# uc-vision/smart-tree

Hardware: AMD Instinct MI355X
Metric: points/sec end-to-end (voxelize->sparse-UNet->skeleton), 1M-pt tree (higher is better)
Workload: dtype f32

## Files before the change

### smart_tree_amd/csrc/brick.hip

```cpp
#include "st_common.h"
#include "st_grid.h"

#define BK_BLOCK 256
#define BK_MAX_DEPTH 6

struct alignas(16) BkRec {
    unsigned long long mask[8];
    unsigned char cum[8];
    unsigned tidx;
    unsigned cum_hi;
};

struct BkLevel {
    int mb;
    unsigned mt;
    int64_t ntab;
    uint32_t* p;
    BkRec* rec;
    uint32_t* base;
    int64_t slot_cap;
    int64_t* n_slots;
    int64_t* n_vox;
};

struct BkState {
    int ext[ST_MAX_SEG][3];
    unsigned fail;
};

__device__ __forceinline__ unsigned bk_spread3(unsigned v) {
    v &= 0x7fu;
    v = (v | (v << 8)) & 0x0000700fu;
    v = (v | (v << 4)) & 0x000430c3u;
    v = (v | (v << 2)) & 0x00049249u;
    return v;
}
__device__ __forceinline__ unsigned bk_compact3(unsigned v) {
    v &= 0x00049249u;
    v = (v | (v >> 2)) & 0x000430c3u;
    v = (v | (v >> 4)) & 0x0000700fu;
    v = (v | (v >> 8)) & 0x0000007fu;
    return v;
}
__device__ __forceinline__ unsigned bk_morton(int bz, int by, int bx) { return (bk_spread3((unsigned)bz) << 2) | (bk_spread3((unsigned)by) << 1) | bk_spread3((unsigned)bx); }
__device__ __forceinline__ unsigned bk_cum(const BkRec& r, int w) { return (unsigned)r.cum[w] + (((r.cum_hi >> w) & 1u) << 8); }

__device__ __forceinline__ int64_t bk_tab(const BkLevel& L, int b, int z, int y, int x) {
    return (int64_t)b * L.mt + bk_morton(z >> 3, y >> 3, x >> 3);
}
__device__ __forceinline__ int bk_lookup(const BkLevel& L, int b, int z, int y, int x) {
    const int lim = 8 << L.mb;
    if ((unsigned)z >= (unsigned)lim || (unsigned)y >= (unsigned)lim || (unsigned)x >= (unsigned)lim) return -1;
    const int64_t t = bk_tab(L, b, z, y, x);
    const uint32_t s = L.p[t];
    if (L.p[t + 1] == s) return -1;
    const BkRec& r = L.rec[s];
    const int w = z & 7, bit = ((y & 7) << 3) | (x & 7);
    const unsigned long long m = r.mask[w];
    if (!((m >> bit) & 1ull)) return -1;
    return (int)(L.base[s] + bk_cum(r, w) + (unsigned)__popcll(m & ((1ull << bit) - 1ull)));
}

#define BK_LOOP(i, n) for (int64_t i = (int64_t)blockIdx.x * blockDim.x + threadIdx.x; i < (n); i += (int64_t)gridDim.x * blockDim.x)

static inline unsigned bk_grid(int64_t n) {
    int64_t g = st_div_up(n > 0 ? n : 1, BK_BLOCK);
    return (unsigned)(g < 16384 ? g : 16384);
}

__global__ void __launch_bounds__(BK_BLOCK) k_bk_mark0(const int32_t* coords, int64_t n, BkLevel L, BkState* st, const int32_t* blk_seg,
                                                       int nseg, int nblk) {
    __shared__ int m[ST_MAX_SEG * 3];
    for (int i = threadIdx.x; i < nseg * 3; i += blockDim.x) m[i] = 0;
    __syncthreads();
    const int lim = 8 << L.mb;
    BK_LOOP(i, n) {
        const int4 c = reinterpret_cast<const int4*>(coords)[i];
        if ((unsigned)c.x >= (unsigned)nblk || (unsigned)c.y >= (unsigned)lim || (unsigned)c.z >= (unsigned)lim || (unsigned)c.w >= (unsigned)lim) {
            atomicOr(&st->fail, 2u);
            continue;
        }
        L.p[bk_tab(L, c.x, c.y, c.z, c.w)] = 1u;
        const int s = blk_seg ? blk_seg[c.x] : 0;
        if (c.y > m[3 * s]) atomicMax(&m[3 * s], c.y);
        if (c.z > m[3 * s + 1]) atomicMax(&m[3 * s + 1], c.z);
        if (c.w > m[3 * s + 2]) atomicMax(&m[3 * s + 2], c.w);
    }
    __syncthreads();
    for (int i = threadIdx.x; i < nseg * 3; i += blockDim.x) if (m[i]) atomicMax(&(&st->ext[0][0])[i], m[i]);
}

__global__ void __launch_bounds__(BK_BLOCK) k_bk_init_rec(BkLevel L, BkState* st) {
    BK_LOOP(t, L.ntab) {
        const uint32_t s = L.p[t];
        if (L.p[t + 1] == s) continue;
        if ((int64_t)s >= L.slot_cap) { atomicOr(&st->fail, 1u); continue; }
        BkRec r;
#pragma unroll
        for (int w = 0; w < 8; w++) { r.mask[w] = 0ull; r.cum[w] = 0; }
        r.tidx = (unsigned)t;
        r.cum_hi = 0u;
        L.rec[s] = r;
    }
}

__device__ __forceinline__ void bk_set_bit(const BkLevel& L, int b, int z, int y, int x) {
    const uint32_t s = L.p[bk_tab(L, b, z, y, x)];
    if ((int64_t)s >= L.slot_cap) return;
    const int bit = ((y & 7) << 3) | (x & 7);
    unsigned* half = reinterpret_cast<unsigned*>(&L.rec[s].mask[z & 7]) + (bit >> 5);
    const unsigned v = 1u << (bit & 31);
    if (!(*half & v)) atomicOr(half, v);
}

__global__ void __launch_bounds__(BK_BLOCK) k_bk_bits0(const int32_t* coords, int64_t n, BkLevel L, const BkState* st) {
    if (st->fail) return;
    const int lim = 8 << L.mb;
    BK_LOOP(i, n) {
        const int4 c = reinterpret_cast<const int4*>(coords)[i];
        if ((unsigned)c.y >= (unsigned)lim || (unsigned)c.z >= (unsigned)lim || (unsigned)c.w >= (unsigned)lim) continue;
        bk_set_bit(L, c.x, c.y, c.z, c.w);
    }
}

__global__ void __launch_bounds__(BK_BLOCK) k_bk_count(BkLevel L) {
    const int64_t ns = *L.n_slots < L.slot_cap ? *L.n_slots : L.slot_cap;
    BK_LOOP(s, ns) {
        BkRec& r = L.rec[s];
        unsigned run = 0, hi = 0;
#pragma unroll
        for (int w = 0; w < 8; w++) {
            r.cum[w] = (unsigned char)(run & 255u);
            hi |= (run >> 8) << w;
            run += (unsigned)__popcll(r.mask[w]);
        }
        r.cum_hi = hi;
        L.base[s] = run;
    }
}

__global__ void __launch_bounds__(BK_BLOCK) k_bk_order0(const int32_t* coords, int64_t n, BkLevel L, int32_t* order0, int32_t* sorted,
                                                        const BkState* st) {
    if (st->fail) return;
    BK_LOOP(i, n) {
        const int4 c = reinterpret_cast<const int4*>(coords)[i];
        const int r = bk_lookup(L, c.x, c.y, c.z, c.w);
        if (r < 0 || r >= n) continue;
        order0[r] = (int32_t)i;
        reinterpret_cast<int4*>(sorted)[r] = c;
    }
}

__global__ void __launch_bounds__(BK_BLOCK) k_bk_subm(const int32_t* coords, const int64_t* n_dev, int64_t cap, BkLevel L, int32_t* nbr,
                                                      const BkState* st) {
    if (st->fail) return;
    const int64_t n = *n_dev < cap ? *n_dev : cap;
    const int lim = 8 << L.mb;
    BK_LOOP(o, n) {
        const int4 c = reinterpret_cast<const int4*>(coords)[o];
        const int b = c.x, z = c.y, y = c.z, x = c.w;
        int slot[8];
        uint32_t bs[8];
#pragma unroll
        for (int q = 0; q < 8; q++) {
            const int zz = z + ((q & 4) ? 1 : -1), yy = y + ((q & 2) ? 1 : -1), xx = x + ((q & 1) ? 1 : -1);
            slot[q] = -1;
            bs[q] = 0u;
            if ((unsigned)zz < (unsigned)lim && (unsigned)yy < (unsigned)lim && (unsigned)xx < (unsigned)lim) {
                const int64_t t = bk_tab(L, b, zz, yy, xx);
                const uint32_t s = L.p[t];
                if (L.p[t + 1] != s) { slot[q] = (int)s; bs[q] = L.base[s]; }
            }
        }
#pragma unroll
        for (int dz = -1; dz <= 1; dz++) {
            const int zz = z + dz, w = zz & 7;
            const int qz = (zz >> 3) == ((z - 1) >> 3) ? 0 : 4;
            unsigned long long m[4];
            unsigned cu[4];
#pragma unroll
            for (int q = 0; q < 4; q++) {
                const int s = slot[qz | q];
                m[q] = 0ull;
                cu[q] = 0u;
                if (s >= 0 && (unsigned)zz < (unsigned)lim) { const BkRec& r = L.rec[s]; m[q] = r.mask[w]; cu[q] = bs[qz | q] + bk_cum(r, w); }
            }
#pragma unroll
            for (int j = 0; j < 9; j++) {
                const int dy = j / 3 - 1, dx = j % 3 - 1;
                const int yy = y + dy, xx = x + dx, k = (dz + 1) * 9 + j;
                int r = -1;
                if (dz == 0 && j == 4) r = (int)o;
                else if ((unsigned)yy < (unsigned)lim && (unsigned)xx < (unsigned)lim) {
                    const int q = ((yy >> 3) == ((y - 1) >> 3) ? 0 : 2) | ((xx >> 3) == ((x - 1) >> 3) ? 0 : 1);
                    const int bit = ((yy & 7) << 3) | (xx & 7);
                    const unsigned long long mm = m[q];
                    if ((mm >> bit) & 1ull) r = (int)(cu[q] + (unsigned)__popcll(mm & ((1ull << bit) - 1ull)));
                }
                nbr[(int64_t)k * cap + o] = r;
            }
        }
    }
}

__global__ void __launch_bounds__(BK_BLOCK) k_bk_coarse_mark(BkLevel Lf, BkLevel Lc, const BkState* st, int level, const int32_t* blk_seg) {
    if (st->fail) return;
    const int64_t ns = *Lf.n_slots < Lf.slot_cap ? *Lf.n_slots : Lf.slot_cap;
    const int nbc = 1 << Lc.mb;
    BK_LOOP(s, ns) {
        const BkRec& r = Lf.rec[s];
        const unsigned t = r.tidx, mc = t & (Lf.mt - 1u);
        const int b = (int)(t >> (3 * Lf.mb));
        const int fb[3] = {(int)bk_compact3(mc >> 2), (int)bk_compact3(mc >> 1), (int)bk_compact3(mc)};
        const int* e = st->ext[blk_seg ? blk_seg[b] : 0];
        unsigned long long all = 0ull;
#pragma unroll
        for (int w = 0; w < 8; w++) all |= r.mask[w];
        for (int q = 0; q < 8; q++) {
            const int d[3] = {(q >> 2) & 1, (q >> 1) & 1, q & 1};
            unsigned long long m = d[0] ? r.mask[7] : all;
            if (d[1]) m &= 0xff00000000000000ull;
            if (d[2]) m &= 0x8080808080808080ull;
            bool ok = m != 0ull;
            int cb[3];
#pragma unroll
            for (int a = 0; a < 3; a++) {
                cb[a] = (fb[a] >> 1) + d[a];
                ok = ok && (!d[a] || (fb[a] & 1)) && cb[a] < nbc && 8 * cb[a] <= ((e[a] >> level) >> 1);
            }
            if (ok) Lc.p[(int64_t)b * Lc.mt + bk_morton(cb[0], cb[1], cb[2])] = 1u;
        }
    }
}

__global__ void __launch_bounds__(BK_BLOCK) k_bk_coarse_stencil(BkLevel Lf, BkLevel Lc, const BkState* st, int level, const int32_t* blk_seg) {
    if (st->fail) return;
    const int64_t ns = *Lc.n_slots < Lc.slot_cap ? *Lc.n_slots : Lc.slot_cap;
    const int limf = 8 << Lf.mb, nbf = 1 << Lf.mb;
    BK_LOOP(idx, ns * 8) {
        const int64_t s = idx >> 3;
        const int w = (int)(idx & 7);
        const unsigned t = Lc.rec[s].tidx, mc = t & (Lc.mt - 1u);
        const int b = (int)(t >> (3 * Lc.mb));
        const int cb[3] = {(int)bk_compact3(mc >> 2), (int)bk_compact3(mc >> 1), (int)bk_compact3(mc)};
        const int* e = st->ext[blk_seg ? blk_seg[b] : 0];
        const int omax[3] = {(e[0] >> level) >> 1, (e[1] >> level) >> 1, (e[2] >> level) >> 1};
        const int oz = 8 * cb[0] + w;
        unsigned long long word = 0ull;
        if (oz <= omax[0]) {
            unsigned rows[17];
#pragma unroll
            for (int r = 0; r < 17; r++) rows[r] = 0u;
            for (int dz = -1; dz <= 1; dz++) {
                const int fz = 2 * oz + dz;
                if (fz < 0 || fz >= limf) continue;
                const int fbz = fz >> 3, wz = fz & 7;
                for (int iy = 0; iy < 3; iy++) {
                    const int fby = 2 * cb[1] - 1 + iy;
                    if (fby < 0 || fby >= nbf) continue;
                    for (int ix = 0; ix < 3; ix++) {
                        const int fbx = 2 * cb[2] - 1 + ix;
                        if (fbx < 0 || fbx >= nbf) continue;
                        const int64_t tf = (int64_t)b * Lf.mt + bk_morton(fbz, fby, fbx);
                        const uint32_t sf = Lf.p[tf];
                        if (Lf.p[tf + 1] == sf) continue;
                        const unsigned long long m = Lf.rec[sf].mask[wz];
                        if (m == 0ull) continue;
                        for (int yy = iy == 0 ? 7 : 0; yy < 8; yy++) {
                            const unsigned rb = (unsigned)(m >> (8 * yy)) & 0xffu;
                            const int r = iy == 0 ? 0 : (iy == 1 ? 1 + yy : 9 + yy);
                            rows[r] |= ix == 0 ? (rb >> 7) : (ix == 1 ? rb << 1 : rb << 9);
                        }
                    }
                }
            }
            unsigned c8[17];
#pragma unroll
            for (int r = 0; r < 17; r++) {
                unsigned x = rows[r] | (rows[r] >> 1) | (rows[r] >> 2);
                x &= 0x5555u;
                x = (x | (x >> 1)) & 0x3333u;
                x = (x | (x >> 2)) & 0x0f0fu;
                x = (x | (x >> 4)) & 0x00ffu;
                c8[r] = x;
            }
            unsigned xclip = 0xffu;
            if (8 * cb[2] + 7 > omax[2]) xclip = omax[2] >= 8 * cb[2] ? (0xffu >> (7 - (omax[2] - 8 * cb[2]))) : 0u;
#pragma unroll
            for (int oy = 0; oy < 8; oy++) {
                if (8 * cb[1] + oy > omax[1]) break;
                const unsigned rb = (c8[2 * oy] | c8[2 * oy + 1] | c8[2 * oy + 2]) & xclip;
                word |= (unsigned long long)rb << (8 * oy);
            }
        }
        Lc.rec[s].mask[w] = word;
    }
}

__global__ void __launch_bounds__(BK_BLOCK) k_bk_emit(BkLevel L, int32_t* coords, int64_t cap, BkState* st) {
    if (st->fail) return;
    const int64_t ns = *L.n_slots < L.slot_cap ? *L.n_slots : L.slot_cap;
    BK_LOOP(idx, ns * 8) {
        const int64_t s = idx >> 3;
        const int w = (int)(idx & 7);
        const BkRec& r = L.rec[s];
        unsigned long long m = r.mask[w];
        if (m == 0ull) continue;
        const unsigned t = r.tidx, mc = t & (L.mt - 1u);
        const int b = (int)(t >> (3 * L.mb));
        const int z = (int)(bk_compact3(mc >> 2) << 3) | w, y0 = (int)(bk_compact3(mc >> 1) << 3), x0 = (int)(bk_compact3(mc) << 3);
        int64_t row = (int64_t)L.base[s] + bk_cum(r, w);
        while (m) {
            const int bit = __ffsll((long long)m) - 1;
            m &= m - 1ull;
            if (row < cap) reinterpret_cast<int4*>(coords)[row] = make_int4(b, z, y0 + (bit >> 3), x0 + (bit & 7));
            else atomicOr(&st->fail, 1u);
            row++;
        }
    }
}

__device__ __forceinline__ int bk_parity_class(int z, int y, int x) { return ((z & 1) << 2) | ((y & 1) << 1) | (x & 1); }
__global__ void __launch_bounds__(BK_BLOCK) k_bk_updown(const int32_t* coords, const int64_t* n_dev, int64_t cap_f, BkLevel Lc, const BkState* st,
                                                        int level, const int32_t* blk_seg, const int64_t* m_dev, int64_t cap_c,
                                                        int32_t* nbr_up, int32_t* nbr_down, uint32_t* parity_count) {
    __shared__ uint32_t hist[8];
    if (st->fail) return;
    if (threadIdx.x < 8) hist[threadIdx.x] = 0;
    __syncthreads();
    const int64_t n = *n_dev < cap_f ? *n_dev : cap_f;
    const int64_t m = *m_dev < cap_c ? *m_dev : cap_c;
    BK_LOOP(i, n) {
        const int4 c4 = reinterpret_cast<const int4*>(coords)[i];
        const int b = c4.x, c[3] = {c4.y, c4.z, c4.w};
        const int* e = st->ext[blk_seg ? blk_seg[b] : 0];
        const int omax[3] = {(e[0] >> level) >> 1, (e[1] >> level) >> 1, (e[2] >> level) >> 1};
        atomicAdd(&hist[bk_parity_class(c[0], c[1], c[2])], 1u);
        int64_t t_have = -1;
        int slot = -1, w_have = -1;
        unsigned bs = 0u, cu = 0u;
        unsigned long long mw = 0ull;
        const int limc = 8 << Lc.mb;
#pragma unroll
        for (int kz = 0; kz < 3; kz++)
#pragma unroll
            for (int j = 0; j < 9; j++) {
                const int k = kz * 9 + j;
                const int nz = c[0] + 1 - kz, ny = c[1] + 1 - j / 3, nx = c[2] + 1 - j % 3;
                int r = -1;
                if (!((nz | ny | nx) & 1) && nz >= 0 && ny >= 0 && nx >= 0 && (nz >> 1) <= omax[0] && (ny >> 1) <= omax[1] && (nx >> 1) <= omax[2]) {
                    const int oz = nz >> 1, oy = ny >> 1, ox = nx >> 1;
                    if (oz < limc && oy < limc && ox < limc) {
                        const int64_t tc = bk_tab(Lc, b, oz, oy, ox);
                        if (tc != t_have) {
                            t_have = tc;
                            w_have = -1;
                            const uint32_t sc = Lc.p[tc];
                            slot = Lc.p[tc + 1] != sc ? (int)sc : -1;
                            bs = slot >= 0 ? Lc.base[slot] : 0u;
                        }
                        if (slot >= 0) {
                            const int wz = oz & 7;
                            if (wz != w_have) { w_have = wz; const BkRec& rc = Lc.rec[slot]; mw = rc.mask[wz]; cu = bs + bk_cum(rc, wz); }
                            const int bit = ((oy & 7) << 3) | (ox & 7);
                            if ((mw >> bit) & 1ull) r = (int)(cu + (unsigned)__popcll(mw & ((1ull << bit) - 1ull)));
                        }
                    }
                }
                nbr_up[(int64_t)k * cap_f + i] = r;
                if (r >= 0 && r < m) nbr_down[(int64_t)k * cap_c + r] = (int32_t)i;
            }
    }
    __syncthreads();
    if (threadIdx.x < 8 && hist[threadIdx.x]) atomicAdd(&parity_count[threadIdx.x], hist[threadIdx.x]);
}

#define BK_ORDER_BLOCKS 512
__global__ void __launch_bounds__(BK_BLOCK) k_bk_parity_order(const int32_t* coords, const int64_t* n_dev, int64_t cap, const uint32_t* count,
                                                              uint32_t* cursor, int32_t* order, const BkState* st) {
    __shared__ uint32_t hist[8], gbase[8], lcur[8];
    if (st->fail) return;
    const int64_t n = *n_dev < cap ? *n_dev : cap;
    const int lane = threadIdx.x & 63;
    const int64_t per = (n + gridDim.x - 1) / gridDim.x, chunk = (per + BK_BLOCK - 1) / BK_BLOCK * BK_BLOCK;
    const int64_t lo = (int64_t)blockIdx.x * chunk, hi = lo + chunk < n ? lo + chunk : n;
    if (threadIdx.x < 8) { hist[threadIdx.x] = 0; lcur[threadIdx.x] = 0; }
    __syncthreads();
    for (int64_t i0 = lo + (threadIdx.x - lane); i0 < hi; i0 += BK_BLOCK) {
        const int64_t i = i0 + lane;
        int cls = -1;
        if (i < hi) cls = bk_parity_class(coords[4 * i + 1], coords[4 * i + 2], coords[4 * i + 3]);
        for (int q = 0; q < 8; q++) {
            const unsigned long long mask = __ballot(cls == q);
            if (mask != 0ull && lane == __ffsll((long long)mask) - 1) atomicAdd(&hist[q], (uint32_t)__popcll(mask));
        }
    }
    __syncthreads();
    if (threadIdx.x < 8) {
        uint32_t base = 0;
        for (int q = 0; q < (int)threadIdx.x; q++) base += count[q];
        gbase[threadIdx.x] = base + (hist[threadIdx.x] ? atomicAdd(&cursor[threadIdx.x], hist[threadIdx.x]) : 0u);
    }
    __syncthreads();
    for (int64_t i0 = lo + (threadIdx.x - lane); i0 < hi; i0 += BK_BLOCK) {
        const int64_t i = i0 + lane;
        int cls = -1;
        if (i < hi) cls = bk_parity_class(coords[4 * i + 1], coords[4 * i + 2], coords[4 * i + 3]);
        for (int q = 0; q < 8; q++) {
            const unsigned long long mask = __ballot(cls == q);
            if (mask == 0ull) continue;
            const int leader = __ffsll((long long)mask) - 1;
            uint32_t at = 0;
            if (lane == leader) at = atomicAdd(&lcur[q], (uint32_t)__popcll(mask));
            at = __shfl(at, leader);
            if (cls == q)
                order[gbase[q] + at + (uint32_t)__popcll(mask & ((1ull << lane) - 1ull))] = (int32_t)((uint32_t)i | ((8u + (uint32_t)q) << 28));
        }
    }
}

struct BkPlan {
    int depth;
    int mb[BK_MAX_DEPTH + 1];
    int64_t ntab[BK_MAX_DEPTH + 1], slot_cap[BK_MAX_DEPTH + 1];
};

static bool bk_plan(int64_t n0, int n_blocks, int coord_bound, int depth, const int64_t* caps, BkPlan* P) {
    if (depth < 0 || depth > BK_MAX_DEPTH || n_blocks < 1 || coord_bound < 1) return false;
    P->depth = depth;
    int bound = coord_bound;
    for (int l = 0; l <= depth; l++) {
        int nb = (bound + 7) / 8, mb = 0;
        while ((1 << mb) < nb) mb++;
        if (mb > 7) return false;
        P->mb[l] = mb;
        P->ntab[l] = (int64_t)n_blocks << (3 * mb);
        if (P->ntab[l] >= (1ll << 31)) return false;
        const int64_t cap = l == 0 ? n0 : caps[l];
        P->slot_cap[l] = cap < P->ntab[l] ? cap : P->ntab[l];
        bound = (bound - 1) / 2 + 1;
    }
    return true;
}

struct BkLayout {
    BkState* st;
    int64_t* counts;
    uint32_t* p[BK_MAX_DEPTH + 1];
    BkRec* rec[BK_MAX_DEPTH + 1];
    uint32_t* base[BK_MAX_DEPTH + 1];
    char* scan_ws;
    int64_t scan_bytes;
};

static void bk_layout(StArena& a, const BkPlan& P, BkLayout* Y) {
    Y->st = a.take<BkState>(1);
    Y->counts = a.take<int64_t>(2 * (BK_MAX_DEPTH + 1));
    int64_t scan_n = 1;
    for (int l = 0; l <= P.depth; l++) {
        Y->p[l] = a.take<uint32_t>(P.ntab[l] + 1);
        Y->rec[l] = a.take<BkRec>(P.slot_cap[l]);
        Y->base[l] = a.take<uint32_t>(P.slot_cap[l] + 1);
        if (P.ntab[l] + 1 > scan_n) scan_n = P.ntab[l] + 1;
        if (P.slot_cap[l] + 1 > scan_n) scan_n = P.slot_cap[l] + 1;
    }
    Y->scan_bytes = st_scan_ws_bytes(scan_n);
    Y->scan_ws = a.take<char>(Y->scan_bytes);
}

extern "C" int64_t st_brick_pyramid_workspace_bytes(int64_t n0, int n_blocks, int coord_bound, int depth, const int64_t* caps) {
    BkPlan P;
    if (!bk_plan(n0 > 0 ? n0 : 1, n_blocks, coord_bound, depth, caps, &P)) return 0;
    StArena a(nullptr, 0);
    BkLayout Y;
    bk_layout(a, P, &Y);
    return a.used;
}

extern "C" int st_brick_pyramid(const int32_t* coords0, int64_t n0, int n_blocks, int coord_bound, int depth, const int32_t* blk_seg,
                                int nseg, const int64_t* caps, int32_t* order0, int32_t* const* coords_out, int32_t* const* subm,
                                int32_t* const* down, int32_t* const* up, int32_t* const* up_order, int64_t* counts_host, void* ws,
                                int64_t ws_bytes, void* stream_) {
    hipStream_t stream = (hipStream_t)stream_;
    for (int l = 0; l <= depth && l <= BK_MAX_DEPTH; l++) counts_host[l] = 0;
    if (n0 <= 0) return ST_OK;
    ST_REQUIRE(nseg >= 1 && nseg <= ST_MAX_SEG && (nseg == 1 || blk_seg), "brick pyramid: 1 <= clouds per batch <= %d", ST_MAX_SEG);
    ST_REQUIRE(caps && caps[0] >= n0, "brick pyramid: caps[0] must hold the input voxels");
    if (nseg == 1) blk_seg = nullptr;
    BkPlan P;
    ST_REQUIRE(bk_plan(n0, n_blocks, coord_bound, depth, caps, &P), "brick pyramid: cannot be sized for %d blocks of %d^3 cells", n_blocks, coord_bound);
    StArena a(ws, ws_bytes);
    BkLayout Y;
    bk_layout(a, P, &Y);
    if (!a.ok() || !Y.scan_ws) {
        st_set_error("brick pyramid: workspace too small (%lld < %lld)", (long long)ws_bytes, (long long)a.used);
        return ST_ERR_WORKSPACE;
    }
    (void)hipMemsetAsync(Y.st, 0, sizeof(BkState), stream);
    (void)hipMemsetAsync(Y.counts, 0, 2 * (BK_MAX_DEPTH + 1) * sizeof(int64_t), stream);
    BkLevel L[BK_MAX_DEPTH + 1];
    for (int l = 0; l <= depth; l++) {
        L[l].mb = P.mb[l]; L[l].mt = 1u << (3 * P.mb[l]); L[l].ntab = P.ntab[l]; L[l].p = Y.p[l]; L[l].rec = Y.rec[l];
        L[l].base = Y.base[l]; L[l].slot_cap = P.slot_cap[l]; L[l].n_slots = &Y.counts[2 * l]; L[l].n_vox = &Y.counts[2 * l + 1];
        (void)hipMemsetAsync(Y.p[l], 0, (P.ntab[l] + 1) * sizeof(uint32_t), stream);
    }
    auto close_flags = [&](int l) -> int {
        ST_TRY(st_exclusive_scan_u32(L[l].p, L[l].p, L[l].ntab + 1, reinterpret_cast<uint32_t*>(L[l].n_slots), Y.scan_ws, Y.scan_bytes, stream));
        hipLaunchKernelGGL(k_bk_init_rec, dim3(bk_grid(L[l].ntab)), dim3(BK_BLOCK), 0, stream, L[l], Y.st);
        return ST_OK;
    };
    auto close_bits = [&](int l) -> int {
        hipLaunchKernelGGL(k_bk_count, dim3(bk_grid(L[l].slot_cap)), dim3(BK_BLOCK), 0, stream, L[l]);
        ST_TRY(st_exclusive_scan_u32(L[l].base, L[l].base, L[l].slot_cap, reinterpret_cast<uint32_t*>(L[l].n_vox), Y.scan_ws, Y.scan_bytes,
                                     stream, L[l].n_slots));
        return ST_OK;
    };
    hipLaunchKernelGGL(k_bk_mark0, dim3(bk_grid(n0)), dim3(BK_BLOCK), 0, stream, coords0, n0, L[0], Y.st, blk_seg, nseg, n_blocks);
    ST_TRY(close_flags(0));
    hipLaunchKernelGGL(k_bk_bits0, dim3(bk_grid(n0)), dim3(BK_BLOCK), 0, stream, coords0, n0, L[0], (const BkState*)Y.st);
    ST_TRY(close_bits(0));
    hipLaunchKernelGGL(k_bk_order0, dim3(bk_grid(n0)), dim3(BK_BLOCK), 0, stream, coords0, n0, L[0], order0, coords_out[0], (const BkState*)Y.st);
    for (int l = 0;; l++) {
        const int64_t cap = caps[l];
        hipLaunchKernelGGL(k_bk_subm, dim3(bk_grid(cap)), dim3(BK_BLOCK), 0, stream, (const int32_t*)coords_out[l], (const int64_t*)L[l].n_vox, cap,
                           L[l], subm[l], (const BkState*)Y.st);
        if (l == depth) break;
        const int64_t cap_c = caps[l + 1];
        hipLaunchKernelGGL(k_bk_coarse_mark, dim3(bk_grid(L[l].slot_cap)), dim3(BK_BLOCK), 0, stream, L[l], L[l + 1], (const BkState*)Y.st, l, blk_seg);
        ST_TRY(close_flags(l + 1));
        hipLaunchKernelGGL(k_bk_coarse_stencil, dim3(bk_grid(L[l + 1].slot_cap * 8)), dim3(BK_BLOCK), 0, stream, L[l], L[l + 1], (const BkState*)Y.st, l,
                           blk_seg);
        ST_TRY(close_bits(l + 1));
        hipLaunchKernelGGL(k_bk_emit, dim3(bk_grid(L[l + 1].slot_cap * 8)), dim3(BK_BLOCK), 0, stream, L[l + 1], coords_out[l + 1], cap_c, Y.st);
        (void)hipMemsetAsync(down[l], 0xff, 27 * cap_c * sizeof(int32_t), stream);
        uint32_t* pc = reinterpret_cast<uint32_t*>(up_order[l] + cap);
        (void)hipMemsetAsync(pc, 0, 16 * sizeof(uint32_t), stream);
        hipLaunchKernelGGL(k_bk_updown, dim3(bk_grid(cap)), dim3(BK_BLOCK), 0, stream, (const int32_t*)coords_out[l], (const int64_t*)L[l].n_vox, cap,
                           L[l + 1], (const BkState*)Y.st, l, blk_seg, (const int64_t*)L[l + 1].n_vox, cap_c, up[l], down[l], pc);
        const unsigned og = bk_grid(cap) < BK_ORDER_BLOCKS ? bk_grid(cap) : BK_ORDER_BLOCKS;
        hipLaunchKernelGGL(k_bk_parity_order, dim3(og), dim3(BK_BLOCK), 0, stream, (const int32_t*)coords_out[l], (const int64_t*)L[l].n_vox, cap,
                           (const uint32_t*)pc, pc + 8, up_order[l], (const BkState*)Y.st);
    }
    struct { int64_t counts[2 * (BK_MAX_DEPTH + 1)]; } hc;
    unsigned hfail = 0;
    (void)hipMemcpyAsync(&hc, Y.counts, sizeof(hc), hipMemcpyDeviceToHost, stream);
    (void)hipMemcpyAsync(&hfail, &Y.st->fail, sizeof(unsigned), hipMemcpyDeviceToHost, stream);
    st_stream_wait(stream);
    ST_CHECK_LAUNCH();
    ST_REQUIRE(!(hfail & 2u), "brick pyramid: a coordinate lies outside the declared bounds (%d blocks, %d cells per axis)", n_blocks, coord_bound);
    for (int l = 0; l <= depth; l++) counts_host[l] = hc.counts[2 * l + 1];
    bool over = (hfail & 1u) != 0;
    for (int l = 0; l <= depth; l++) over = over || hc.counts[2 * l + 1] > caps[l] || hc.counts[2 * l] > P.slot_cap[l];
    if (over) {
        st_set_error("brick pyramid: a level needs more rows than its capacity (caps)");
        return ST_ERR_WORKSPACE;
    }
    ST_REQUIRE(hc.counts[1] == n0, "brick pyramid: %lld distinct voxels among %lld input rows (duplicate coordinates)", (long long)hc.counts[1],
               (long long)n0);
    return ST_OK;
}
```

Before: 921.4 million.

## Restructure brick pyramid build: fused stencil-count, gather-based down maps, single init kernel

The coarse stencil kernel now also computes per-slot popcount prefix sums (cum, cum_hi, base) with wave shuffles, so the separate count kernel is dropped. For small coarse tables it walks the hash table directly and skips the separate record-init kernel. The down-neighbour map is built by a gather kernel (the subm window kernel templated with doubled coordinates), which replaces the scattered writes and the 27*cap memset. Several memsets are merged into one init kernel. Together these cut launches and memory traffic, at the cost of an extra full window pass over coarse voxels.

```diff
diff --git a/smart_tree_amd/csrc/brick.hip b/smart_tree_amd/csrc/brick.hip
--- a/smart_tree_amd/csrc/brick.hip
+++ b/smart_tree_amd/csrc/brick.hip
@@ -151,14 +151,15 @@
     }
 }
 
-__global__ void __launch_bounds__(BK_BLOCK) k_bk_subm(const int32_t* coords, const int64_t* n_dev, int64_t cap, BkLevel L, int32_t* nbr,
-                                                      const BkState* st) {
+template <bool DOWN>
+__global__ void __launch_bounds__(BK_BLOCK) k_bk_window(const int32_t* coords, const int64_t* n_dev, int64_t cap, BkLevel L, int32_t* nbr,
+                                                        const BkState* st) {
     if (st->fail) return;
     const int64_t n = *n_dev < cap ? *n_dev : cap;
     const int lim = 8 << L.mb;
     BK_LOOP(o, n) {
         const int4 c = reinterpret_cast<const int4*>(coords)[o];
-        const int b = c.x, z = c.y, y = c.z, x = c.w;
+        const int b = c.x, z = DOWN ? 2 * c.y : c.y, y = DOWN ? 2 * c.z : c.z, x = DOWN ? 2 * c.w : c.w;
         int slot[8];
         uint32_t bs[8];
 #pragma unroll
@@ -190,7 +191,7 @@
                 const int dy = j / 3 - 1, dx = j % 3 - 1;
                 const int yy = y + dy, xx = x + dx, k = (dz + 1) * 9 + j;
                 int r = -1;
-                if (dz == 0 && j == 4) r = (int)o;
+                if (!DOWN && dz == 0 && j == 4) r = (int)o;
                 else if ((unsigned)yy < (unsigned)lim && (unsigned)xx < (unsigned)lim) {
                     const int q = ((yy >> 3) == ((y - 1) >> 3) ? 0 : 2) | ((xx >> 3) == ((x - 1) >> 3) ? 0 : 1);
                     const int bit = ((yy & 7) << 3) | (xx & 7);
@@ -233,67 +234,112 @@
     }
 }
 
-__global__ void __launch_bounds__(BK_BLOCK) k_bk_coarse_stencil(BkLevel Lf, BkLevel Lc, const BkState* st, int level, const int32_t* blk_seg) {
-    if (st->fail) return;
+__device__ __forceinline__ unsigned long long bk_stencil_word(const BkLevel& Lf, int b, const int* cb, int w, const int* omax) {
+    const int limf = 8 << Lf.mb, nbf = 1 << Lf.mb;
+    const int oz = 8 * cb[0] + w;
+    unsigned long long word = 0ull;
+    if (oz > omax[0]) return word;
+    unsigned rows[17];
+#pragma unroll
+    for (int r = 0; r < 17; r++) rows[r] = 0u;
+    for (int dz = -1; dz <= 1; dz++) {
+        const int fz = 2 * oz + dz;
+        if (fz < 0 || fz >= limf) continue;
+        const int fbz = fz >> 3, wz = fz & 7;
+        for (int iy = 0; iy < 3; iy++) {
+            const int fby = 2 * cb[1] - 1 + iy;
+            if (fby < 0 || fby >= nbf) continue;
+            for (int ix = 0; ix < 3; ix++) {
+                const int fbx = 2 * cb[2] - 1 + ix;
+                if (fbx < 0 || fbx >= nbf) continue;
+                const int64_t tf = (int64_t)b * Lf.mt + bk_morton(fbz, fby, fbx);
+                const uint32_t sf = Lf.p[tf];
+                if (Lf.p[tf + 1] == sf) continue;
+                const unsigned long long m = Lf.rec[sf].mask[wz];
+                if (m == 0ull) continue;
+                for (int yy = iy == 0 ? 7 : 0; yy < 8; yy++) {
+                    const unsigned rb = (unsigned)(m >> (8 * yy)) & 0xffu;
+                    const int r = iy == 0 ? 0 : (iy == 1 ? 1 + yy : 9 + yy);
+                    rows[r] |= ix == 0 ? (rb >> 7) : (ix == 1 ? rb << 1 : rb << 9);
+                }
+            }
+        }
+    }
+    unsigned c8[17];
+#pragma unroll
+    for (int r = 0; r < 17; r++) {
+        unsigned x = rows[r] | (rows[r] >> 1) | (rows[r] >> 2);
+        x &= 0x5555u;
+        x = (x | (x >> 1)) & 0x3333u;
+        x = (x | (x >> 2)) & 0x0f0fu;
+        x = (x | (x >> 4)) & 0x00ffu;
+        c8[r] = x;
+    }
+    unsigned xclip = 0xffu;
+    if (8 * cb[2] + 7 > omax[2]) xclip = omax[2] >= 8 * cb[2] ? (0xffu >> (7 - (omax[2] - 8 * cb[2]))) : 0u;
+#pragma unroll
+    for (int oy = 0; oy < 8; oy++) {
+        if (8 * cb[1] + oy > omax[1]) break;
+        const unsigned rb = (c8[2 * oy] | c8[2 * oy + 1] | c8[2 * oy + 2]) & xclip;
+        word |= (unsigned long long)rb << (8 * oy);
+    }
+    return word;
+}
+
+#define BK_TABLE_WALK_MAX (1 << 17)
+__global__ void __launch_bounds__(BK_BLOCK) k_bk_coarse_stencil(BkLevel Lf, BkLevel Lc, BkState* st, int level, const int32_t* blk_seg, int by_table) {
+    __shared__ unsigned failed;
+    if (threadIdx.x == 0) failed = st->fail;
+    __syncthreads();
+    if (failed) return;
     const int64_t ns = *Lc.n_slots < Lc.slot_cap ? *Lc.n_slots : Lc.slot_cap;
-    const int limf = 8 << Lf.mb, nbf = 1 << Lf.mb;
-    BK_LOOP(idx, ns * 8) {
-        const int64_t s = idx >> 3;
-        const int w = (int)(idx & 7);
-        const unsigned t = Lc.rec[s].tidx, mc = t & (Lc.mt - 1u);
-        const int b = (int)(t >> (3 * Lc.mb));
-        const int cb[3] = {(int)bk_compact3(mc >> 2), (int)bk_compact3(mc >> 1), (int)bk_compact3(mc)};
-        const int* e = st->ext[blk_seg ? blk_seg[b] : 0];
-        const int omax[3] = {(e[0] >> level) >> 1, (e[1] >> level) >> 1, (e[2] >> level) >> 1};
-        const int oz = 8 * cb[0] + w;
+    const int64_t n8 = (by_table ? Lc.ntab : ns) * 8;
+    const int lane = threadIdx.x & 63, w = threadIdx.x & 7;
+    for (int64_t i0 = (int64_t)blockIdx.x * BK_BLOCK; i0 < n8; i0 += (int64_t)gridDim.x * BK_BLOCK) {
+        const int64_t e8 = (i0 + threadIdx.x) >> 3;
+        int64_t t = 0;
+        uint32_t s = 0u;
+        bool live = e8 * 8 < n8;
+        if (live && by_table) {
+            t = e8;
+            s = Lc.p[t];
+            live = Lc.p[t + 1] != s;
+            if (live && (int64_t)s >= Lc.slot_cap) {
+                if (w == 0) atomicOr(&st->fail, 1u);
+                live = false;
+            }
+        } else if (live) {
+            s = (uint32_t)e8;
+            t = Lc.rec[s].tidx;
+        }
         unsigned long long word = 0ull;
-        if (oz <= omax[0]) {
-            unsigned rows[17];
-#pragma unroll
-            for (int r = 0; r < 17; r++) rows[r] = 0u;
-            for (int dz = -1; dz <= 1; dz++) {
-                const int fz = 2 * oz + dz;
-                if (fz < 0 || fz >= limf) continue;
-                const int fbz = fz >> 3, wz = fz & 7;
-                for (int iy = 0; iy < 3; iy++) {
-                    const int fby = 2 * cb[1] - 1 + iy;
-                    if (fby < 0 || fby >= nbf) continue;
-                    for (int ix = 0; ix < 3; ix++) {
-                        const int fbx = 2 * cb[2] - 1 + ix;
-                        if (fbx < 0 || fbx >= nbf) continue;
-                        const int64_t tf = (int64_t)b * Lf.mt + bk_morton(fbz, fby, fbx);
-                        const uint32_t sf = Lf.p[tf];
-                        if (Lf.p[tf + 1] == sf) continue;
-                        const unsigned long long m = Lf.rec[sf].mask[wz];
-                        if (m == 0ull) continue;
-                        for (int yy = iy == 0 ? 7 : 0; yy < 8; yy++) {
-                            const unsigned rb = (unsigned)(m >> (8 * yy)) & 0xffu;
-                            const int r = iy == 0 ? 0 : (iy == 1 ? 1 + yy : 9 + yy);
-                            rows[r] |= ix == 0 ? (rb >> 7) : (ix == 1 ? rb << 1 : rb << 9);
-                        }
-                    }
-                }
-            }
-            unsigned c8[17];
-#pragma unroll
-            for (int r = 0; r < 17; r++) {
-                unsigned x = rows[r] | (rows[r] >> 1) | (rows[r] >> 2);
-                x &= 0x5555u;
-                x = (x | (x >> 1)) & 0x3333u;
-                x = (x | (x >> 2)) & 0x0f0fu;
-                x = (x | (x >> 4)) & 0x00ffu;
-                c8[r] = x;
-            }
-            unsigned xclip = 0xffu;
-            if (8 * cb[2] + 7 > omax[2]) xclip = omax[2] >= 8 * cb[2] ? (0xffu >> (7 - (omax[2] - 8 * cb[2]))) : 0u;
-#pragma unroll
-            for (int oy = 0; oy < 8; oy++) {
-                if (8 * cb[1] + oy > omax[1]) break;
-                const unsigned rb = (c8[2 * oy] | c8[2 * oy + 1] | c8[2 * oy + 2]) & xclip;
-                word |= (unsigned long long)rb << (8 * oy);
-            }
-        }
-        Lc.rec[s].mask[w] = word;
+        if (live) {
+            const unsigned mc = (unsigned)t & (Lc.mt - 1u);
+            const int b = (int)((unsigned)t >> (3 * Lc.mb));
+            const int cb[3] = {(int)bk_compact3(mc >> 2), (int)bk_compact3(mc >> 1), (int)bk_compact3(mc)};
+            const int* e = st->ext[blk_seg ? blk_seg[b] : 0];
+            const int omax[3] = {(e[0] >> level) >> 1, (e[1] >> level) >> 1, (e[2] >> level) >> 1};
+            word = bk_stencil_word(Lf, b, cb, w, omax);
+        }
+        const unsigned pop = (unsigned)__popcll(word);
+        unsigned run = pop;
+#pragma unroll
+        for (int d = 1; d < 8; d <<= 1) {
+            const unsigned v = __shfl_up(run, (unsigned)d, 8);
+            if (w >= d) run += v;
+        }
+        const unsigned before = run - pop;
+        const unsigned long long big = __ballot(before >= 256u);
+        if (live) {
+            BkRec& r = Lc.rec[s];
+            r.mask[w] = word;
+            r.cum[w] = (unsigned char)(before & 255u);
+            if (w == 7) {
+                r.tidx = (unsigned)t;
+                r.cum_hi = (unsigned)(big >> (lane & ~7)) & 0xffu;
+                Lc.base[s] = run;
+            }
+        }
     }
 }
 
@@ -321,15 +367,13 @@
 }
 
 __device__ __forceinline__ int bk_parity_class(int z, int y, int x) { return ((z & 1) << 2) | ((y & 1) << 1) | (x & 1); }
-__global__ void __launch_bounds__(BK_BLOCK) k_bk_updown(const int32_t* coords, const int64_t* n_dev, int64_t cap_f, BkLevel Lc, const BkState* st,
-                                                        int level, const int32_t* blk_seg, const int64_t* m_dev, int64_t cap_c,
-                                                        int32_t* nbr_up, int32_t* nbr_down, uint32_t* parity_count) {
+__global__ void __launch_bounds__(BK_BLOCK) k_bk_up(const int32_t* coords, const int64_t* n_dev, int64_t cap_f, BkLevel Lc, const BkState* st,
+                                                        int level, const int32_t* blk_seg, int32_t* nbr_up, uint32_t* parity_count) {
     __shared__ uint32_t hist[8];
     if (st->fail) return;
     if (threadIdx.x < 8) hist[threadIdx.x] = 0;
     __syncthreads();
     const int64_t n = *n_dev < cap_f ? *n_dev : cap_f;
-    const int64_t m = *m_dev < cap_c ? *m_dev : cap_c;
     BK_LOOP(i, n) {
         const int4 c4 = reinterpret_cast<const int4*>(coords)[i];
         const int b = c4.x, c[3] = {c4.y, c4.z, c4.w};
@@ -368,7 +412,6 @@
                     }
                 }
                 nbr_up[(int64_t)k * cap_f + i] = r;
-                if (r >= 0 && r < m) nbr_down[(int64_t)k * cap_c + r] = (int32_t)i;
             }
     }
     __syncthreads();
@@ -417,6 +460,18 @@
                 order[gbase[q] + at + (uint32_t)__popcll(mask & ((1ull << lane) - 1ull))] = (int32_t)((uint32_t)i | ((8u + (uint32_t)q) << 28));
         }
     }
+}
+
+struct BkZero {
+    uint32_t* pc[BK_MAX_DEPTH];
+    int depth;
+};
+__global__ void __launch_bounds__(BK_BLOCK) k_bk_init(BkState* st, int64_t* counts, BkZero z) {
+    uint32_t* s = reinterpret_cast<uint32_t*>(st);
+    for (unsigned i = threadIdx.x; i < sizeof(BkState) / sizeof(uint32_t); i += blockDim.x) s[i] = 0u;
+    for (unsigned i = threadIdx.x; i < 2 * (BK_MAX_DEPTH + 1); i += blockDim.x) counts[i] = 0;
+    if (threadIdx.x < 16)
+        for (int l = 0; l < z.depth; l++) z.pc[l][threadIdx.x] = 0u;
 }
 
 struct BkPlan {
@@ -496,50 +551,51 @@
         st_set_error("brick pyramid: workspace too small (%lld < %lld)", (long long)ws_bytes, (long long)a.used);
         return ST_ERR_WORKSPACE;
     }
-    (void)hipMemsetAsync(Y.st, 0, sizeof(BkState), stream);
-    (void)hipMemsetAsync(Y.counts, 0, 2 * (BK_MAX_DEPTH + 1) * sizeof(int64_t), stream);
+    BkZero Z;
+    Z.depth = depth;
+    for (int l = 0; l < BK_MAX_DEPTH; l++) Z.pc[l] = l < depth ? reinterpret_cast<uint32_t*>(up_order[l] + caps[l]) : nullptr;
+    hipLaunchKernelGGL(k_bk_init, dim3(1), dim3(BK_BLOCK), 0, stream, Y.st, Y.counts, Z);
     BkLevel L[BK_MAX_DEPTH + 1];
     for (int l = 0; l <= depth; l++) {
         L[l].mb = P.mb[l]; L[l].mt = 1u << (3 * P.mb[l]); L[l].ntab = P.ntab[l]; L[l].p = Y.p[l]; L[l].rec = Y.rec[l];
         L[l].base = Y.base[l]; L[l].slot_cap = P.slot_cap[l]; L[l].n_slots = &Y.counts[2 * l]; L[l].n_vox = &Y.counts[2 * l + 1];
         (void)hipMemsetAsync(Y.p[l], 0, (P.ntab[l] + 1) * sizeof(uint32_t), stream);
     }
-    auto close_flags = [&](int l) -> int {
-        ST_TRY(st_exclusive_scan_u32(L[l].p, L[l].p, L[l].ntab + 1, reinterpret_cast<uint32_t*>(L[l].n_slots), Y.scan_ws, Y.scan_bytes, stream));
-        hipLaunchKernelGGL(k_bk_init_rec, dim3(bk_grid(L[l].ntab)), dim3(BK_BLOCK), 0, stream, L[l], Y.st);
-        return ST_OK;
+    auto scan_flags = [&](int l) -> int {
+        return st_exclusive_scan_u32(L[l].p, L[l].p, L[l].ntab + 1, reinterpret_cast<uint32_t*>(L[l].n_slots), Y.scan_ws, Y.scan_bytes, stream);
     };
-    auto close_bits = [&](int l) -> int {
-        hipLaunchKernelGGL(k_bk_count, dim3(bk_grid(L[l].slot_cap)), dim3(BK_BLOCK), 0, stream, L[l]);
-        ST_TRY(st_exclusive_scan_u32(L[l].base, L[l].base, L[l].slot_cap, reinterpret_cast<uint32_t*>(L[l].n_vox), Y.scan_ws, Y.scan_bytes,
-                                     stream, L[l].n_slots));
-        return ST_OK;
+    auto scan_base = [&](int l) -> int {
+        return st_exclusive_scan_u32(L[l].base, L[l].base, L[l].slot_cap, reinterpret_cast<uint32_t*>(L[l].n_vox), Y.scan_ws, Y.scan_bytes, stream,
+                                     L[l].n_slots);
     };
     hipLaunchKernelGGL(k_bk_mark0, dim3(bk_grid(n0)), dim3(BK_BLOCK), 0, stream, coords0, n0, L[0], Y.st, blk_seg, nseg, n_blocks);
-    ST_TRY(close_flags(0));
+    ST_TRY(scan_flags(0));
+    hipLaunchKernelGGL(k_bk_init_rec, dim3(bk_grid(L[0].ntab)), dim3(BK_BLOCK), 0, stream, L[0], Y.st);
     hipLaunchKernelGGL(k_bk_bits0, dim3(bk_grid(n0)), dim3(BK_BLOCK), 0, stream, coords0, n0, L[0], (const BkState*)Y.st);
-    ST_TRY(close_bits(0));
+    hipLaunchKernelGGL(k_bk_count, dim3(bk_grid(L[0].slot_cap)), dim3(BK_BLOCK), 0, stream, L[0]);
+    ST_TRY(scan_base(0));
     hipLaunchKernelGGL(k_bk_order0, dim3(bk_grid(n0)), dim3(BK_BLOCK), 0, stream, coords0, n0, L[0], order0, coords_out[0], (const BkState*)Y.st);
     for (int l = 0;; l++) {
         const int64_t cap = caps[l];
-        hipLaunchKernelGGL(k_bk_subm, dim3(bk_grid(cap)), dim3(BK_BLOCK), 0, stream, (const int32_t*)coords_out[l], (const int64_t*)L[l].n_vox, cap,
+        hipLaunchKernelGGL(k_bk_window<false>, dim3(bk_grid(cap)), dim3(BK_BLOCK), 0, stream, (const int32_t*)coords_out[l], (const int64_t*)L[l].n_vox, cap,
                            L[l], subm[l], (const BkState*)Y.st);
         if (l == depth) break;
         const int64_t cap_c = caps[l + 1];
         hipLaunchKernelGGL(k_bk_coarse_mark, dim3(bk_grid(L[l].slot_cap)), dim3(BK_BLOCK), 0, stream, L[l], L[l + 1], (const BkState*)Y.st, l, blk_seg);
-        ST_TRY(close_flags(l + 1));
-        hipLaunchKernelGGL(k_bk_coarse_stencil, dim3(bk_grid(L[l + 1].slot_cap * 8)), dim3(BK_BLOCK), 0, stream, L[l], L[l + 1], (const BkState*)Y.st, l,
-                           blk_seg);
-        ST_TRY(close_bits(l + 1));
+        ST_TRY(scan_flags(l + 1));
+        const bool by_table = L[l + 1].ntab <= BK_TABLE_WALK_MAX;
+        if (!by_table) hipLaunchKernelGGL(k_bk_init_rec, dim3(bk_grid(L[l + 1].ntab)), dim3(BK_BLOCK), 0, stream, L[l + 1], Y.st);
+        hipLaunchKernelGGL(k_bk_coarse_stencil, dim3(bk_grid((by_table ? L[l + 1].ntab : L[l + 1].slot_cap) * 8)), dim3(BK_BLOCK), 0, stream, L[l],
+                           L[l + 1], Y.st, l, blk_seg, by_table ? 1 : 0);
+        ST_TRY(scan_base(l + 1));
         hipLaunchKernelGGL(k_bk_emit, dim3(bk_grid(L[l + 1].slot_cap * 8)), dim3(BK_BLOCK), 0, stream, L[l + 1], coords_out[l + 1], cap_c, Y.st);
-        (void)hipMemsetAsync(down[l], 0xff, 27 * cap_c * sizeof(int32_t), stream);
-        uint32_t* pc = reinterpret_cast<uint32_t*>(up_order[l] + cap);
-        (void)hipMemsetAsync(pc, 0, 16 * sizeof(uint32_t), stream);
-        hipLaunchKernelGGL(k_bk_updown, dim3(bk_grid(cap)), dim3(BK_BLOCK), 0, stream, (const int32_t*)coords_out[l], (const int64_t*)L[l].n_vox, cap,
-                           L[l + 1], (const BkState*)Y.st, l, blk_seg, (const int64_t*)L[l + 1].n_vox, cap_c, up[l], down[l], pc);
+        hipLaunchKernelGGL(k_bk_window<true>, dim3(bk_grid(cap_c)), dim3(BK_BLOCK), 0, stream, (const int32_t*)coords_out[l + 1],
+                           (const int64_t*)L[l + 1].n_vox, cap_c, L[l], down[l], (const BkState*)Y.st);
+        hipLaunchKernelGGL(k_bk_up, dim3(bk_grid(cap)), dim3(BK_BLOCK), 0, stream, (const int32_t*)coords_out[l], (const int64_t*)L[l].n_vox, cap,
+                           L[l + 1], (const BkState*)Y.st, l, blk_seg, up[l], Z.pc[l]);
         const unsigned og = bk_grid(cap) < BK_ORDER_BLOCKS ? bk_grid(cap) : BK_ORDER_BLOCKS;
         hipLaunchKernelGGL(k_bk_parity_order, dim3(og), dim3(BK_BLOCK), 0, stream, (const int32_t*)coords_out[l], (const int64_t*)L[l].n_vox, cap,
-                           (const uint32_t*)pc, pc + 8, up_order[l], (const BkState*)Y.st);
+                           (const uint32_t*)Z.pc[l], Z.pc[l] + 8, up_order[l], (const BkState*)Y.st);
     }
     struct { int64_t counts[2 * (BK_MAX_DEPTH + 1)]; } hc;
     unsigned hfail = 0;
```

After: 920.8 million. Within noise of the previous version (-0.1%).
